# jmaronas/TGP.pytorch

Hardware: AMD Instinct MI355X
Metric: ELBO-steps/sec (N x M kernel + chol + flow), Power M=100 S=32 (higher is better)
Workload: dtype f64; 1 GPU; tgp_power_tanh3x2; rows_per_gpu=8611, D=4, M=100, S=32, flow=tanh3x2, parallelism=row-shard x1, launch=hipgraph, 40 / 10 steps per graph launch, replicas=1

## Files before the change

tgp/pytorch_amd/csrc/tgp_rows.hpp:

```cpp
#pragma once
#include "tgp_dev.hpp"
#include "tgp_prep.hpp"

namespace tgp {

#define TGP_NODES_IN_FLIGHT 4

__device__ __forceinline__ void lds_barrier() { asm volatile("s_waitcnt lgkmcnt(0)\n\ts_barrier" ::: "memory"); }

struct RowArgs {
  Plan p;
  const double* X;
  const double* Y;
  const double* rowp;
  double* g_rowp;
  double* mu;
  double* v;
  double* ws;
  FlowProg prog;
  const double* xs;
  const double* wn;
  double scale;
};

struct RowLds {
  size_t zs, ils, mv, tile, xt, vbs, mbs, tp, tg, ti, xs, wn, stack, acc, red, prog, rin, cbuf, rpl, total;
};
#define TGP_RW_SMALL 10
#define TGP_RW_NODES 5

__host__ __device__ inline RowLds row_lds(const Plan& p, int mode, int nslots, int rw = 16) {
  const bool train = mode != 0;
  RowLds L;
  size_t o = 0;
  auto take = [&o](size_t n) { size_t r = o; o += (n + 1) / 2 * 2; return r; };
  L.zs = take((size_t)p.MP * p.DP);
  L.ils = take(16);
  L.mv = take(p.MP);
  L.tp = take(p.P + 1);
  L.tg = take(p.P + 1);
  L.ti = take(p.P + 1);
  L.xs = take(p.S + 1);
  L.wn = take(p.S + 1);
  L.prog = take((size_t)2 * p.nblk + 2);
  L.red = take(32);
  if (train) {
    L.tile = take((size_t)p.MP * TGP_TILE_LD);
    L.xt = take((size_t)TGP_ROWS_PER_BLOCK * p.CT16);
    L.vbs = take(TGP_ROWS_PER_BLOCK);
    L.mbs = take(TGP_ROWS_PER_BLOCK);
    const size_t st = (size_t)(nslots > 0 ? nslots : 1) * (mode == 1 ? (rw < 16 ? TGP_RW_NODES : TGP_NODES_IN_FLIGHT) : 1) * 256;
    if (L.tile + st > o) take(L.tile + st - o);
    L.stack = L.tile;
    L.acc = take((size_t)(p.P > 0 ? p.P : 1) * 64 + (size_t)p.RP * 256);
    L.rin = L.cbuf = L.rpl = o;
    if (rw < 16) {
      L.rin = take(4 * 48);
      L.cbuf = take((size_t)4 * 64 * TGP_RW_NODES);
      L.rpl = take((size_t)4 * 16 * 2 * p.RP);
    }
  } else {
    L.tile = take((size_t)p.MP * 32);
    L.xt = L.vbs = L.mbs = L.stack = L.acc = L.rin = L.cbuf = L.rpl = o;
  }
  L.total = o;
  return L;
}

template <int MAXSTEPS, class FB>
__device__ __forceinline__ d4 mfma_chain(const double* a0, int step0, int nsteps, FB fb) {
  d4 c = {0, 0, 0, 0};
#pragma unroll
  for (int s0 = 0; s0 < MAXSTEPS; s0 += 8) {
    double av[8];
#pragma unroll
    for (int u = 0; u < 8; ++u)
      if (s0 + u < nsteps) av[u] = a0[(step0 + s0 + u) * 64];
#pragma unroll
    for (int u = 0; u < 8; ++u)
      if (s0 + u < nsteps) c = TGP_MFMA(av[u], fb(s0 + u), c);
    __builtin_amdgcn_sched_group_barrier(0x100, 8, 0);
    __builtin_amdgcn_sched_group_barrier(0x008, 8, 0);
  }
  return c;
}

template <int MAXSTEPS, class FA, class FB>
__device__ __forceinline__ d4 subst_chain(const double* a0, int nsum, int dstep0, d4 c, FA fa, FB fb) {
  d4 out = {0, 0, 0, 0};
#pragma unroll
  for (int s0 = 0; s0 < MAXSTEPS; s0 += 8) {
    double av[8];
#pragma unroll
    for (int u = 0; u < 8; ++u) {
      const int s = s0 + u;
      if (s < nsum) av[u] = a0[fa(s) * 64];
      else if (s < nsum + 4) av[u] = a0[(dstep0 + s - nsum) * 64];
    }
#pragma unroll
    for (int u = 0; u < 8; ++u) {
      const int s = s0 + u;
      if (s < nsum) c = TGP_MFMA(av[u], fb(s), c);
      else if (s < nsum + 4) out = TGP_MFMA(av[u], c[s - nsum], out);
    }
    __builtin_amdgcn_sched_group_barrier(0x100, 8, 0);
    __builtin_amdgcn_sched_group_barrier(0x008, 8, 0);
  }
  return out;
}

#ifdef TGP_STAMPS
#define ROW_STAMP(wsp, plan, i)                                                                       \
  do {                                                                                                \
    if (bid == 0 && threadIdx.x == 0)                                                                 \
      (wsp)[(plan).hdr + tgp::H_STAMP + (i)] = (double)__builtin_amdgcn_s_memrealtime();              \
  } while (0)
#else
#define ROW_STAMP(wsp, plan, i) \
  do {                          \
  } while (0)
#endif

template <int MT, int DP, int MODEX, int RW = 16>
__global__ __launch_bounds__(256) __attribute__((amdgpu_waves_per_eu(1, 1))) void k_rows(RowArgs a) {
  constexpr int MODE = MODEX & (TGP_FLOWX - 1);
  constexpr bool X = MODEX & TGP_FLOWX;
  static_assert(RW == 16 || (RW == TGP_RW_SMALL && MODE == 1), "rows per wave: 16, or TGP_RW_SMALL in training mode 1");
  constexpr bool TRAIN = MODE != 0;
  constexpr int RBK = 4 * RW;
  constexpr int MP = MT * 16;
  constexpr int CT = (2 * DP + 1 + 15) / 16, CT16 = CT * 16;
  constexpr int LD = TGP_TILE_LD;
  extern __shared__ __attribute__((aligned(16))) unsigned char smem_raw[];
  double* sm = reinterpret_cast<double*>(smem_raw);
  const Plan& p = a.p;
  const RowLds L = row_lds(p, MODE, a.prog.nslots, RW);
  double* zs = sm + L.zs;
  double* ils = sm + L.ils;
  double* mv = sm + L.mv;
  double* tpL = sm + L.tp;
  double* tgL = sm + L.tg;
  double* tiL = sm + L.ti;
  double* xsL = sm + L.xs;
  double* wnL = sm + L.wn;
  int32_t* progL = reinterpret_cast<int32_t*>(sm + L.prog);
  double* red = sm + L.red;
  double* tile = sm + L.tile;
  double* xt = sm + L.xt;
  double* vbs = sm + L.vbs;
  double* mbs = sm + L.mbs;
  double* stack = sm + L.stack;
  double* acc = sm + L.acc;

  const int tid = threadIdx.x, lane = tid & 63, wave = tid >> 6, nl = lane & 15, q = lane >> 4;
  const double* __restrict__ ws = a.ws;
  const int N = p.N, D = p.D, M = p.M, P = p.P, RP = p.RP;
  const int bid = blockIdx.x;

  if (TRAIN && bid >= p.nblocks) {
    const int c = __builtin_amdgcn_readfirstlane(bid - p.nblocks);
    const int wv = __builtin_amdgcn_readfirstlane(wave);
    const double* __restrict__ LTg = ws + p.LT;
    const double* __restrict__ nDg = ws + p.nD;
    const double* __restrict__ Sg = ws + p.S_;
    constexpr int NLF = MT > 1 ? MT * (MT - 1) / 2 : 1;
    double lf[NLF][4], df[MT][4];
    d4 Jt[MT];
#pragma unroll
    for (int i = 0; i < MT; ++i) {
      if (i < c) continue;
#pragma unroll
      for (int s4 = 0; s4 < 4; ++s4) df[i][s4] = *(nDg + i * 256 + nl * 16 + 4 * s4 + q);
#pragma unroll
      for (int kb = 0; kb < i; ++kb) {
        if (kb < c) continue;
#pragma unroll
        for (int s4 = 0; s4 < 4; ++s4) lf[i * (i - 1) / 2 + kb][s4] = *(LTg + (size_t)(16 * kb + 4 * s4 + q) * MP + 16 * i + nl);
      }
    }
    d4 dc;
#pragma unroll
    for (int rr = 0; rr < 4; ++rr) dc[rr] = -*(nDg + c * 256 + (4 * rr + q) * 16 + nl);
    double mf[MT][4];
#pragma unroll
    for (int i = 0; i < MT; ++i)
#pragma unroll
      for (int rr = 0; rr < 4; ++rr) mf[i][rr] = *(ws + p.mpad + 16 * i + 4 * rr + q);
#pragma unroll
    for (int i = 0; i < MT; ++i) {
      Jt[i] = d4{0, 0, 0, 0};
      if (i < c) continue;
      if (i == c) { Jt[i] = dc; continue; }
      d4 acc = {0, 0, 0, 0};
#pragma unroll
      for (int kb = 0; kb < i; ++kb) {
        if (kb < c) continue;
#pragma unroll
        for (int s4 = 0; s4 < 4; ++s4) acc = TGP_MFMA(lf[i * (i - 1) / 2 + kb][s4], Jt[kb][s4], acc);
      }
      d4 o = {0, 0, 0, 0};
#pragma unroll
      for (int s4 = 0; s4 < 4; ++s4) o = TGP_MFMA(df[i][s4], acc[s4], o);
      Jt[i] = o;
    }
    if (wv == 0) {
#pragma unroll
      for (int i = 0; i < MT; ++i) {
        if (i < c) continue;
#pragma unroll
        for (int rr = 0; rr < 4; ++rr) a.ws[p.J + (size_t)(16 * i + 4 * rr + q) * MP + 16 * c + nl] = Jt[i][rr];
      }
    }
    for (int jj = wv; jj < MT; jj += 4) {
      double bf[MT][4];
#pragma unroll
      for (int kb = 0; kb < MT; ++kb) {
        if (kb < c) continue;
#pragma unroll
        for (int s4 = 0; s4 < 4; ++s4) {
          const int kk = 16 * kb + 4 * s4 + q;
          bf[kb][s4] = *(Sg + (size_t)kk * MP + 16 * jj + nl) - (kk == 16 * jj + nl ? 1.0 : 0.0);
        }
      }
      d4 h = {0, 0, 0, 0};
#pragma unroll
      for (int kb = 0; kb < MT; ++kb) {
        if (kb < c) continue;
#pragma unroll
        for (int s4 = 0; s4 < 4; ++s4) h = TGP_MFMA(Jt[kb][s4], bf[kb][s4], h);
      }
#pragma unroll
      for (int rr = 0; rr < 4; ++rr) a.ws[p.HpT + (size_t)(16 * jj + nl) * MP + 16 * c + 4 * rr + q] = h[rr];
    }
    if (wv == 3) {
      double sw = 0.0;
#pragma unroll
      for (int i = 0; i < MT; ++i) {
        if (i < c) continue;
#pragma unroll
        for (int rr = 0; rr < 4; ++rr) sw += Jt[i][rr] * mf[i][rr];
      }
      sw = quad_sum(sw);
      if (q == 0) a.ws[p.w + 16 * c + nl] = sw;
    }
    return;
  }

  ROW_STAMP(a.ws, p, 0);
#ifdef TGP_STAMPS
  if (bid == 0 && threadIdx.x == 0) a.ws[p.hdr + H_STAMP + 11] = (double)clock64();
#endif
  const int n = bid * RBK + wave * RW + nl;
  const bool valid = nl < RW && n < N;
  const int nc = valid ? n : N - 1;
  double xraw[DP];
#pragma unroll
  for (int d = 0; d < DP; ++d) xraw[d] = d < D ? a.X[(size_t)nc * D + d] : 0.0;
  const double y = TRAIN ? a.Y[nc] : 0.0;
  double rraw[2] = {0.0, 0.0};
  if constexpr (RW < 16) {
    if (a.rowp != nullptr && RP > 0 && RP <= 8) {
      rraw[0] = q < RP ? a.rowp[(size_t)nc * RP + q] : 0.0;
      rraw[1] = q + 4 < RP ? a.rowp[(size_t)nc * RP + q + 4] : 0.0;
    }
  }
  const double s2 = *(ws + p.hdr + H_S2), eta = *(ws + p.hdr + H_ETA),
               einv = *(ws + p.hdr + H_EINV);

  const double* __restrict__ LTm = ws + p.LT;
  const double* __restrict__ Lm = ws + p.L;
  const double* __restrict__ nD = ws + p.nD;
  const double* __restrict__ Lq = ws + p.Lq;
  const double* __restrict__ LqT = ws + p.LqT;
  double* pan = tile;
  double stg[2][MT];
  auto issue = [&](int kind, int i, double (&st)[MT]) {
    const bool lower = kind == 0 || kind == 2;
    const double* __restrict__ Mt = (kind == 0 ? LTm : (kind == 1 ? Lq : (kind == 2 ? LqT : Lm))) +
                                    (size_t)((lower ? 0 : 16 * i) + (tid >> 4)) * MP + 16 * i + (tid & 15);
    const int nb = lower ? i + 1 : MT - i;
#pragma unroll
    for (int u = 0; u < MT; ++u)
      if (u < nb) {
        if (kind == 0 && u == i) st[u] = *(nD + i * 256 + (tid & 15) * 16 + (tid >> 4));
        else if (kind == 3 && u == 0) st[u] = *(nD + i * 256 + (tid >> 4) * 16 + (tid & 15));
        else st[u] = *(Mt + (size_t)16 * u * MP);
      }
  };
  auto commit = [&](int par, bool lower, int i, const double (&st)[MT]) {
    const int nb = lower ? i + 1 : MT - i;
    double* buf = pan + par * (MP * 16) + ((lower ? 0 : 16 * i) + (tid >> 4)) * 16 + (tid & 15);
#pragma unroll
    for (int u = 0; u < MT; ++u)
      if (u < nb) buf[16 * u * 16] = st[u];
  };
  auto issue1 = [&](int pp, double (&st)[MT]) { if (pp < MT) issue(0, pp, st); else issue(1, pp - MT, st); };
  auto issue2 = [&](int pp, double (&st)[MT]) { if (pp < MT) issue(2, pp, st); else issue(3, 2 * MT - 1 - pp, st); };
  issue1(0, stg[0]);
  if (MT * 2 > 1) issue1(1, stg[1]);
  {
    constexpr int NZ = (MP * DP + 255) / 256;
    double zv[NZ];
#pragma unroll
    for (int u = 0; u < NZ; ++u) zv[u] = tid + 256 * u < MP * DP ? *(ws + p.Zs + tid + 256 * u) : 0.0;
    const double mv0 = tid < MP ? *(ws + p.mpad + tid) : 0.0;
    const double il0 = tid < 16 ? *(ws + p.ils + tid) : 0.0;
    const bool fl = p.lik == TGP_LIK_FLOW;
    const double tp0 = (fl && tid < P) ? *(ws + p.tp + tid) : 0.0, tg0 = (fl && tid < P) ? *(ws + p.tg + tid) : 0.0;
    const double xs0 = (fl && tid < p.S) ? a.xs[tid] : 0.0, wn0 = (fl && tid < p.S) ? a.wn[tid] : 0.0;
#pragma unroll
    for (int u = 0; u < NZ; ++u)
      if (tid + 256 * u < MP * DP) zs[tid + 256 * u] = zv[u];
    if (tid < MP) mv[tid] = mv0;
    if (tid < 16) ils[tid] = il0;
    if (fl) {
      if (tid < P) { tpL[tid] = tp0; tgL[tid] = tg0; tiL[tid] = rcp_fast(tp0); }
      if (tid < p.S) { xsL[tid] = xs0; wnL[tid] = wn0; }
      for (int i = tid + 256; i < P; i += 256) { tpL[i] = *(ws + p.tp + i); tgL[i] = *(ws + p.tg + i); tiL[i] = rcp_fast(tpL[i]); }
      for (int i = tid + 256; i < p.S; i += 256) { xsL[i] = a.xs[i]; wnL[i] = a.wn[i]; }
      for (int i = tid; i < 4 * p.nblk; i += 256) progL[i] = a.prog.blk[i];
    }
  }
  if (TRAIN) {
    const int nacc = P * 64 + RP * 256;
    for (int i = tid; i < nacc; i += 256) acc[i] = 0.0;
  }
  lds_barrier();

  ROW_STAMP(a.ws, p, 1);
  double x[DP];
#pragma unroll
  for (int d = 0; d < DP; ++d) x[d] = d < D ? xraw[d] * ils[d] : 0.0;


  double Kr[4 * MT];
#pragma unroll
  for (int k0 = 0; k0 < 4 * MT; k0 += 4) {
    double e[4];
    TGP_EACH(u, 4) {
      const int mm = 4 * (k0 + u) + q;
      double d2 = 0.0;
#pragma unroll
      for (int d = 0; d < DP; ++d) {
        const double t = x[d] - zs[mm * DP + d];
        d2 += t * t;
      }
      e[u] = -0.5 * d2;
    }
    exp_fast_n<4>(e);
    TGP_EACH(u, 4) Kr[k0 + u] = (4 * (k0 + u) + q < M ? s2 : 0.0) * e[u];
  }

  ROW_STAMP(a.ws, p, 2);
  d4 Aa[MT], Ba[MT];
#pragma unroll
  for (int i = 0; i < MT; ++i) {
    const double* buf = pan + (i & 1) * (MP * 16);
    commit(i & 1, true, i, stg[i & 1]);
    lds_barrier();
    if (i + 2 < 2 * MT) issue1(i + 2, stg[i & 1]);
    const d4 c0 = {-Kr[4 * i], -Kr[4 * i + 1], -Kr[4 * i + 2], -Kr[4 * i + 3]};
    Aa[i] = subst_chain<4 * MT>(buf + q * 16 + nl, 4 * i, 4 * i, c0, [&](int st) { return st; },
                                [&](int st) { return Aa[st / 4][st % 4]; });
  }
  ROW_STAMP(a.ws, p, 3);
#pragma unroll
  for (int i = 0; i < MT; ++i) {
    const double* buf = pan + ((MT + i) & 1) * (MP * 16);
    commit((MT + i) & 1, false, i, stg[(MT + i) & 1]);
    lds_barrier();
    if (MT + i + 2 < 2 * MT) issue1(MT + i + 2, stg[(MT + i) & 1]);
    Ba[i] = mfma_chain<4 * MT>(buf + q * 16 + nl, 4 * i, 4 * (MT - i), [&](int st) { return Aa[i + st / 4][st % 4]; });
  }
  ROW_STAMP(a.ws, p, 4);
  double pm = 0.0, pa = 0.0, pb = 0.0;
#pragma unroll
  for (int i = 0; i < MT; ++i)
#pragma unroll
    for (int r = 0; r < 4; ++r) {
      pm += mv[16 * i + 4 * r + q] * Aa[i][r];
      pa += Aa[i][r] * Aa[i][r];
      pb += Ba[i][r] * Ba[i][r];
    }
  pm = quad_sum(pm); pa = quad_sum(pa); pb = quad_sum(pb);
  const double mu = pm, v = s2 - pa + pb;
  if (a.mu != nullptr && q == 0 && valid) { a.mu[n] = mu; a.v[n] = v; }
  if (!TRAIN) return;

  ROW_STAMP(a.ws, p, 5);
  double mub = 0.0, vb = 0.0, ellp = 0.0, etap = 0.0;
  if (p.lik == TGP_LIK_GAUSS) {
    const double r = y - mu;
    mub = a.scale * einv * r;
    vb = -0.5 * a.scale * einv;
    if (q == 0) {
      ellp = -0.5 * TGP_LOG_2PI_REF - 0.5 * eta - 0.5 * einv * (r * r + v);
      etap = -0.5 + 0.5 * einv * (r * r + v);
    }
  } else if (p.lik == TGP_LIK_ADJOINT) {
    mub = y;
    vb = a.rowp[nc];
  } else {
    FlowDev F{progL, p.nblk, tpL, tgL, tiL};
    const double sq = sqrt(2.0 * v);
    if constexpr (RW < 16) {
      constexpr int NB = TGP_RW_NODES;
      double* rin = sm + L.rin + wave * 48;
      double* cb = sm + L.cbuf + wave * (64 * NB);
      if (q == 0) { rin[nl] = mu; rin[16 + nl] = sq; rin[32 + nl] = y; }
      double* rpl = sm + L.rpl + wave * (16 * 2 * RP);
      if (a.rowp != nullptr && RP > 0 && nl < RW) {
        for (int col = q; col < RP; col += 4) {
          const double raw = RP <= 8 ? rraw[col >> 2] : a.rowp[(size_t)nc * RP + col];
          double val = raw, der = 1.0;
          for (int b = 0; b < p.nblk; ++b) {
            const int kind = progL[4 * b], poff = progL[4 * b + 2], flags = progL[4 * b + 3];
            if ((flags & TGP_FLAG_PER_ROW) && (flags & TGP_FLAG_RESTRICT) && col == poff + (kind == TGP_FLOW_AFFINE ? 0 : 1)) {
              val = softplus_d(raw);
              der = sigmoid_d(raw);
            }
          }
          rpl[(nl * RP + col) * 2] = val;
          rpl[(nl * RP + col) * 2 + 1] = der;
        }
      }
      double* accq = acc + wave * 16 + nl;
      double* accr = acc + (size_t)P * 64 + tid;
      lds_barrier();
      double xn[NB], wq[NB], f[NB], c[NB], yv[NB];
      const double* rpn[NB];
#pragma unroll
      for (int u = 0; u < NB; ++u) {
        const int pp = lane + 64 * u, row = pp % RW, sn = pp / RW;
        const int nr = bid * RBK + wave * RW + row;
        const bool ok = sn < p.S && nr < N;
        xn[u] = xsL[sn < p.S ? sn : 0];
        wq[u] = ok ? wnL[sn < p.S ? sn : 0] : 0.0;
        f[u] = rin[row] + rin[16 + row] * xn[u];
        yv[u] = rin[32 + row];
        rpn[u] = rpl + row * RP * 2;
      }
      flow_forward_store<NB, true, X>(F, f, nullptr, stack + tid, 256, rpn);
#pragma unroll
      for (int u = 0; u < NB; ++u) {
        const double r = yv[u] - f[u];
        ellp += wq[u] * (-0.5 * TGP_LOG_2PI_REF - 0.5 * eta - 0.5 * einv * r * r);
        etap += wq[u] * (-0.5 + 0.5 * einv * r * r);
        c[u] = a.scale * einv * wq[u] * r;
      }
      flow_backward_store<NB, 0, true, X>(F, c, nullptr, stack + tid, 256, a.prog.nslots, accq, 64, q == 0, accr, 256, rpn, stack + tid);
#pragma unroll
      for (int u = 0; u < NB; ++u) cb[lane + 64 * u] = c[u];
      __builtin_amdgcn_fence(__ATOMIC_RELEASE, "wavefront");
      __builtin_amdgcn_wave_barrier();
      if (a.g_rowp != nullptr && RP > 0) {
        int sl = 0;
        for (int b = 0; b < p.nblk; ++b) {
          const int kind = progL[4 * b], K = progL[4 * b + 1], poff = progL[4 * b + 2], flags = progL[4 * b + 3];
          if (kind == TGP_FLOW_SAL && (flags & TGP_FLAG_PER_ROW)) {
#pragma unroll
            for (int jj = 0; jj < 2; ++jj) {
              double gsum = 0.0;
              if (nl < RW) {
                for (int sn = q; sn < p.S; sn += 4) {
                  const int pp = sn * RW + nl;
                  gsum += stack[((sl + jj) * NB + (pp >> 6)) * 256 + wave * 64 + (pp & 63)];
                }
              }
              gsum = quad_sum(gsum);
              if (q == 0 && valid) a.g_rowp[(size_t)n * RP + poff + jj] = gsum;
            }
          }
          sl += flow_block_slots<X>(kind, K);
        }
      }
      double cm = 0.0, cv = 0.0;
      if (nl < RW) {
        for (int sn = q; sn < p.S; sn += 4) {
          const double cc = cb[sn * RW + nl];
          cm += cc;
          cv += cc * xsL[sn];
        }
      }
      mub = quad_sum(cm);
      vb = quad_sum(cv) / sq;
      if (!valid) { mub = 0.0; vb = 0.0; }
    } else {
      const double* rp = (a.rowp != nullptr && RP > 0) ? a.rowp + (size_t)nc * RP : nullptr;
      double cm = 0.0, cv = 0.0;
      {
        constexpr int NB = MODE == 1 ? TGP_NODES_IN_FLIGHT : 1;
        double* accq = acc + wave * 16 + nl;
        double* accr = acc + (size_t)P * 64 + tid;
        const int ntrip = (p.S + 4 * NB - 1) / (4 * NB);
        lds_barrier();
        for (int it = 0; it < ntrip; ++it) {
          double xn[NB], wq[NB], f[NB], c[NB];
#pragma unroll
          for (int u = 0; u < NB; ++u) {
            const int sn = q + 4 * (NB * it + u);
            xn[u] = xsL[sn < p.S ? sn : 0];
            wq[u] = (valid && sn < p.S) ? wnL[sn] : 0.0;
            f[u] = mu + sq * xn[u];
          }
          flow_forward_store<NB, false, X>(F, f, rp, stack + tid, 256);
#pragma unroll
          for (int u = 0; u < NB; ++u) {
            const double r = y - f[u];
            ellp += wq[u] * (-0.5 * TGP_LOG_2PI_REF - 0.5 * eta - 0.5 * einv * r * r);
            etap += wq[u] * (-0.5 + 0.5 * einv * r * r);
            c[u] = a.scale * einv * wq[u] * r;
          }
          flow_backward_store<NB, 0, false, X>(F, c, rp, stack + tid, 256, a.prog.nslots, accq, 64, q == 0, accr, 256);
#pragma unroll
          for (int u = 0; u < NB; ++u) {
            cm += c[u];
            cv += c[u] * xn[u];
          }
        }
      }
      mub = quad_sum(cm);
      vb = quad_sum(cv) / sq;
      if (!valid) { mub = 0.0; vb = 0.0; ellp = 0.0; etap = 0.0; }
    }
  }
  if (p.lik != TGP_LIK_FLOW && !valid) { mub = 0.0; vb = 0.0; ellp = 0.0; etap = 0.0; }

  ROW_STAMP(a.ws, p, 6);
#pragma unroll
  for (int i = 0; i < MT; ++i) Ba[i] *= vb;
  d4 Ca[MT];
  lds_barrier();
  issue2(0, stg[0]);
  issue2(1, stg[1]);
#pragma unroll
  for (int i = 0; i < MT; ++i) {
    const double* buf = pan + (i & 1) * (MP * 16);
    commit(i & 1, true, i, stg[i & 1]);
    lds_barrier();
    if (i + 2 < 2 * MT) issue2(i + 2, stg[i & 1]);
    Ca[i] = mfma_chain<4 * MT>(buf + q * 16 + nl, 0, 4 * (i + 1), [&](int st) { return Ba[st / 4][st % 4]; });
  }
#pragma unroll
  for (int i = 0; i < MT; ++i)
#pragma unroll
    for (int r = 0; r < 4; ++r) Ca[i][r] = mv[16 * i + 4 * r + q] * mub - 2.0 * Aa[i][r] * vb + 2.0 * Ca[i][r];
#pragma unroll
  for (int t = 0; t < MT; ++t) {
    const int i = MT - 1 - t, pp = MT + t;
    const double* buf = pan + (pp & 1) * (MP * 16);
    commit(pp & 1, false, i, stg[pp & 1]);
    lds_barrier();
    if (pp + 2 < 2 * MT) issue2(pp + 2, stg[pp & 1]);
    Ba[i] = subst_chain<4 * MT>(buf + q * 16 + nl, 4 * (MT - 1 - i), 4 * i, -Ca[i],
                                [&](int st) { return 4 * (MT - 1 - st / 4) + st % 4; },
                                [&](int st) { return Ba[MT - 1 - st / 4][st % 4]; });
  }
  lds_barrier();

  ROW_STAMP(a.ws, p, 7);
  double* slab = a.ws + p.slabs + (size_t)bid * p.slab_len;
  const int col = wave * RW + nl;

#pragma unroll
  for (int i = 0; i < MT; ++i)
#pragma unroll
    for (int r = 0; r < 4; ++r)
      if (RW == 16 || nl < RW) tile[(16 * i + 4 * r + q) * LD + col] = Ba[i][r] * Kr[4 * i + r];
#pragma unroll
  for (int c = 0; c < CT16; ++c) {
    if ((c & 3) == q && (RW == 16 || nl < RW)) {
      double val = 0.0;
      if (c < DP) val = x[c < DP ? c : 0];
      else if (c < 2 * DP) val = x[(c - DP) < DP ? (c - DP) : 0] * x[(c - DP) < DP ? (c - DP) : 0];
      else if (c == 2 * DP) val = 1.0;
      xt[col * CT16 + c] = val;
    }
  }
  lds_barrier();
  for (int t = wave; t < MT * CT; t += 4) {
    const int ti = t / CT, tc = t % CT;
    d4 c = {0, 0, 0, 0};
    c = tile_mm_f([&](int k) { return tile[(16 * ti + nl) * LD + k + q]; },
                  [&](int k) { return xt[(k + q) * CT16 + 16 * tc + nl]; }, 0, RBK, c);
#pragma unroll
    for (int r = 0; r < 4; ++r) st_wt(&slab[p.slab_T + (size_t)(16 * ti + q + 4 * r) * CT16 + 16 * tc + nl], c[r]);
  }
  lds_barrier();

  ROW_STAMP(a.ws, p, 8);
#pragma unroll
  for (int i = 0; i < MT; ++i)
#pragma unroll
    for (int r = 0; r < 4; ++r)
      if (RW == 16 || nl < RW) tile[(16 * i + 4 * r + q) * LD + col] = Aa[i][r];
  if (q == 0 && (RW == 16 || nl < RW)) { vbs[col] = vb; mbs[col] = mub; }
  lds_barrier();
  ROW_STAMP(a.ws, p, 17);
  {
    const int ngroups = (MT + 1) / 2;
    if (wave < ngroups) {
      int rows[2], nrows;
      if (MT & 1) {
        if (wave == 0) { rows[0] = MT - 1; nrows = 1; }
        else { rows[0] = MT - 1 - wave; rows[1] = wave - 1; nrows = 2; }
      } else {
        rows[0] = MT - 1 - wave; rows[1] = wave; nrows = 2;
      }
      for (int g = 0; g < nrows; ++g) {
        const int ti = rows[g];
        double af[RW];
#pragma unroll
        for (int nk = 0; nk < RW; ++nk) af[nk] = tile[(16 * ti + nl) * LD + 4 * nk + q];
        {
          d4 c = {0, 0, 0, 0};
          double bm[RW];
#pragma unroll
          for (int nk = 0; nk < RW; ++nk) bm[nk] = nl == 0 ? mbs[4 * nk + q] : 0.0;
#pragma unroll
          for (int nk = 0; nk < RW; ++nk) c = TGP_MFMA(af[nk], bm[nk], c);
          if (nl == 0) {
#pragma unroll
            for (int r = 0; r < 4; ++r) st_wt(&slab[p.slab_S + 16 * ti + q + 4 * r], c[r]);
          }
        }
#pragma unroll
        for (int nk = 0; nk < RW; ++nk) af[nk] *= vbs[4 * nk + q];
        for (int tj = 0; tj <= ti; ++tj) {
          const int t = ti * (ti + 1) / 2 + tj;
          d4 c = {0, 0, 0, 0};
#pragma unroll
          for (int h = 0; h < 2; ++h) {
            constexpr int HB = (RW + 1) / 2;
            double bv[HB];
#pragma unroll
            for (int u = 0; u < HB; ++u)
              if (HB * h + u < RW) bv[u] = tile[(16 * tj + nl) * LD + 4 * (HB * h + u) + q];
#pragma unroll
            for (int u = 0; u < HB; ++u)
              if (HB * h + u < RW) c = TGP_MFMA(af[HB * h + u], bv[u], c);
          }
#pragma unroll
          for (int r = 0; r < 4; ++r) st_wt(&slab[p.slab_G + (size_t)t * 256 + (q + 4 * r) * 16 + nl], c[r]);
        }
      }
    }
  }
  ROW_STAMP(a.ws, p, 18);

  ROW_STAMP(a.ws, p, 9);
  const double e1 = wave_sum(ellp), e2 = wave_sum(etap), e3 = wave_sum(q == 0 ? vb : 0.0);
  if (lane == 0) { red[wave * 4] = e1; red[wave * 4 + 1] = e2; red[wave * 4 + 2] = e3; }
  lds_barrier();
  if (tid == 0) {
    st_wt(&slab[p.slab_C + C_ELL], a.scale * (red[0] + red[4] + red[8] + red[12]));
    st_wt(&slab[p.slab_C + C_ETAB], a.scale * (red[1] + red[5] + red[9] + red[13]));
    st_wt(&slab[p.slab_C + C_SVB], red[2] + red[6] + red[10] + red[14]);
    st_wt(&slab[p.slab_C + C_PAD], 0.0);
  }
  for (int j = wave; j < P; j += 4) {
    const double s = wave_sum(acc[j * 64 + lane]);
    if (lane == 0) st_wt(&slab[p.slab_C + C_THETA + j], s);
  }
  ROW_STAMP(a.ws, p, 10);
#ifdef TGP_STAMPS
  if (bid == 0 && threadIdx.x == 0) a.ws[p.hdr + H_STAMP + 23] = (double)clock64();
#endif
  for (size_t i = p.slab_C + C_THETA + P + tid; i < p.slab_len; i += 256) st_wt(&slab[i], 0.0);
  if (RW == 16 && a.g_rowp != nullptr && q == 0 && valid) {
    const double* rbase = acc + (size_t)P * 64;
    for (int jr = 0; jr < RP; ++jr) {
      const double* ap = rbase + (size_t)jr * 256 + wave * 64 + nl;
      a.g_rowp[(size_t)n * RP + jr] = ap[0] + ap[16] + ap[32] + ap[48];
    }
  }
}

}
```

Measured before the change: 10650 ELBO-steps/s.

## Fold Lq·Lqᵀ into precomputed S matrix to drop triangular passes in training

In the training path, the per-row variance term and backward pass no longer run separate Lq and LqT triangular panel sweeps. A precomputed dense matrix S (at ws+p.S_) is applied once to Aa, giving v = s2 + Aa·(S Aa) with an identity subtracted on the diagonal blocks. The backward then reuses that product, so one full panel-streaming loop and its MFMA chains go away. The cost is a dense rather than triangular block loop for the S product, and it relies on S being computed and stored elsewhere, which is not visible here.

```diff
diff --git a/tgp/pytorch_amd/csrc/tgp_rows.hpp b/tgp/pytorch_amd/csrc/tgp_rows.hpp
--- a/tgp/pytorch_amd/csrc/tgp_rows.hpp
+++ b/tgp/pytorch_amd/csrc/tgp_rows.hpp
@@ -270,15 +270,16 @@
   const double* __restrict__ LTm = ws + p.LT;
   const double* __restrict__ Lm = ws + p.L;
   const double* __restrict__ nD = ws + p.nD;
-  const double* __restrict__ Lq = ws + p.Lq;
-  const double* __restrict__ LqT = ws + p.LqT;
+  constexpr int KIND2 = TRAIN ? 2 : 1;
+  const double* __restrict__ Sm = ws + (TRAIN ? p.S_ : p.Lq);
+  const double dg = (tid >> 4) == (tid & 15) ? 1.0 : 0.0;
   double* pan = tile;
   double stg[2][MT];
   auto issue = [&](int kind, int i, double (&st)[MT]) {
-    const bool lower = kind == 0 || kind == 2;
-    const double* __restrict__ Mt = (kind == 0 ? LTm : (kind == 1 ? Lq : (kind == 2 ? LqT : Lm))) +
-                                    (size_t)((lower ? 0 : 16 * i) + (tid >> 4)) * MP + 16 * i + (tid & 15);
-    const int nb = lower ? i + 1 : MT - i;
+    const bool upper = kind == 1 || kind == 3;
+    const double* __restrict__ Mt = (kind == 0 ? LTm : (kind == 3 ? Lm : Sm)) +
+                                    (size_t)((upper ? 16 * i : 0) + (tid >> 4)) * MP + 16 * i + (tid & 15);
+    const int nb = kind == 0 ? i + 1 : (kind == 2 ? MT : MT - i);
 #pragma unroll
     for (int u = 0; u < MT; ++u)
       if (u < nb) {
@@ -287,15 +288,16 @@
         else st[u] = *(Mt + (size_t)16 * u * MP);
       }
   };
-  auto commit = [&](int par, bool lower, int i, const double (&st)[MT]) {
-    const int nb = lower ? i + 1 : MT - i;
-    double* buf = pan + par * (MP * 16) + ((lower ? 0 : 16 * i) + (tid >> 4)) * 16 + (tid & 15);
+  auto commit = [&](int par, int kind, int i, const double (&st)[MT]) {
+    const bool upper = kind == 1 || kind == 3;
+    const int nb = kind == 0 ? i + 1 : (kind == 2 ? MT : MT - i);
+    double* buf = pan + par * (MP * 16) + ((upper ? 16 * i : 0) + (tid >> 4)) * 16 + (tid & 15);
 #pragma unroll
     for (int u = 0; u < MT; ++u)
-      if (u < nb) buf[16 * u * 16] = st[u];
+      if (u < nb) buf[16 * u * 16] = (kind == 2 && u == i) ? st[u] - dg : st[u];
   };
-  auto issue1 = [&](int pp, double (&st)[MT]) { if (pp < MT) issue(0, pp, st); else issue(1, pp - MT, st); };
-  auto issue2 = [&](int pp, double (&st)[MT]) { if (pp < MT) issue(2, pp, st); else issue(3, 2 * MT - 1 - pp, st); };
+  auto issue1 = [&](int pp, double (&st)[MT]) { if (pp < MT) issue(0, pp, st); else issue(KIND2, pp - MT, st); };
+  auto issue2 = [&](int pp, double (&st)[MT]) { issue(3, MT - 1 - pp, st); };
   issue1(0, stg[0]);
   if (MT * 2 > 1) issue1(1, stg[1]);
   {
@@ -352,11 +354,11 @@
   }
 
   ROW_STAMP(a.ws, p, 2);
-  d4 Aa[MT], Ba[MT];
+  d4 Aa[MT], Ca[MT];
 #pragma unroll
   for (int i = 0; i < MT; ++i) {
     const double* buf = pan + (i & 1) * (MP * 16);
-    commit(i & 1, true, i, stg[i & 1]);
+    commit(i & 1, 0, i, stg[i & 1]);
     lds_barrier();
     if (i + 2 < 2 * MT) issue1(i + 2, stg[i & 1]);
     const d4 c0 = {-Kr[4 * i], -Kr[4 * i + 1], -Kr[4 * i + 2], -Kr[4 * i + 3]};
@@ -367,23 +369,26 @@
 #pragma unroll
   for (int i = 0; i < MT; ++i) {
     const double* buf = pan + ((MT + i) & 1) * (MP * 16);
-    commit((MT + i) & 1, false, i, stg[(MT + i) & 1]);
+    commit((MT + i) & 1, KIND2, i, stg[(MT + i) & 1]);
     lds_barrier();
     if (MT + i + 2 < 2 * MT) issue1(MT + i + 2, stg[(MT + i) & 1]);
-    Ba[i] = mfma_chain<4 * MT>(buf + q * 16 + nl, 4 * i, 4 * (MT - i), [&](int st) { return Aa[i + st / 4][st % 4]; });
+    if constexpr (TRAIN) Ca[i] = mfma_chain<4 * MT>(buf + q * 16 + nl, 0, 4 * MT, [&](int st) { return Aa[st / 4][st % 4]; });
+    else
+      Ca[i] = mfma_chain<4 * MT>(buf + q * 16 + nl, 4 * i, 4 * (MT - i), [&](int st) { return Aa[i + st / 4][st % 4]; });
   }
   ROW_STAMP(a.ws, p, 4);
-  double pm = 0.0, pa = 0.0, pb = 0.0;
+  double pm = 0.0, pa = 0.0, pc = 0.0;
 #pragma unroll
   for (int i = 0; i < MT; ++i)
 #pragma unroll
     for (int r = 0; r < 4; ++r) {
       pm += mv[16 * i + 4 * r + q] * Aa[i][r];
-      pa += Aa[i][r] * Aa[i][r];
-      pb += Ba[i][r] * Ba[i][r];
-    }
-  pm = quad_sum(pm); pa = quad_sum(pa); pb = quad_sum(pb);
-  const double mu = pm, v = s2 - pa + pb;
+      if constexpr (TRAIN) pc += Aa[i][r] * Ca[i][r];
+      else { pa += Aa[i][r] * Aa[i][r]; pc += Ca[i][r] * Ca[i][r]; }
+    }
+  pm = quad_sum(pm); pc = quad_sum(pc);
+  if constexpr (!TRAIN) pa = quad_sum(pa);
+  const double mu = pm, v = TRAIN ? s2 + pc : s2 - pa + pc;
   if (a.mu != nullptr && q == 0 && valid) { a.mu[n] = mu; a.v[n] = v; }
   if (!TRAIN) return;
 
@@ -527,32 +532,25 @@
   if (p.lik != TGP_LIK_FLOW && !valid) { mub = 0.0; vb = 0.0; ellp = 0.0; etap = 0.0; }
 
   ROW_STAMP(a.ws, p, 6);
-#pragma unroll
-  for (int i = 0; i < MT; ++i) Ba[i] *= vb;
-  d4 Ca[MT];
+  issue2(0, stg[0]);
+  if (MT > 1) issue2(1, stg[1]);
+  {
+    const double nmub = -mub, nvb2 = -2.0 * vb;
+#pragma unroll
+    for (int i = 0; i < MT; ++i)
+#pragma unroll
+      for (int r = 0; r < 4; ++r) Ca[i][r] = mv[16 * i + 4 * r + q] * nmub + nvb2 * Ca[i][r];
+  }
+  d4 Ba[MT];
   lds_barrier();
-  issue2(0, stg[0]);
-  issue2(1, stg[1]);
-#pragma unroll
-  for (int i = 0; i < MT; ++i) {
-    const double* buf = pan + (i & 1) * (MP * 16);
-    commit(i & 1, true, i, stg[i & 1]);
+#pragma unroll
+  for (int t = 0; t < MT; ++t) {
+    const int i = MT - 1 - t, pp = t;
+    const double* buf = pan + (pp & 1) * (MP * 16);
+    commit(pp & 1, 3, i, stg[pp & 1]);
     lds_barrier();
-    if (i + 2 < 2 * MT) issue2(i + 2, stg[i & 1]);
-    Ca[i] = mfma_chain<4 * MT>(buf + q * 16 + nl, 0, 4 * (i + 1), [&](int st) { return Ba[st / 4][st % 4]; });
-  }
-#pragma unroll
-  for (int i = 0; i < MT; ++i)
-#pragma unroll
-    for (int r = 0; r < 4; ++r) Ca[i][r] = mv[16 * i + 4 * r + q] * mub - 2.0 * Aa[i][r] * vb + 2.0 * Ca[i][r];
-#pragma unroll
-  for (int t = 0; t < MT; ++t) {
-    const int i = MT - 1 - t, pp = MT + t;
-    const double* buf = pan + (pp & 1) * (MP * 16);
-    commit(pp & 1, false, i, stg[pp & 1]);
-    lds_barrier();
-    if (pp + 2 < 2 * MT) issue2(pp + 2, stg[pp & 1]);
-    Ba[i] = subst_chain<4 * MT>(buf + q * 16 + nl, 4 * (MT - 1 - i), 4 * i, -Ca[i],
+    if (pp + 2 < MT) issue2(pp + 2, stg[pp & 1]);
+    Ba[i] = subst_chain<4 * MT>(buf + q * 16 + nl, 4 * (MT - 1 - i), 4 * i, Ca[i],
                                 [&](int st) { return 4 * (MT - 1 - st / 4) + st % 4; },
                                 [&](int st) { return Ba[MT - 1 - st / 4][st % 4]; });
   }
```

New measurement: 10890 ELBO-steps/s (median of 6 runs). 1.02x the previous value.
